# WangChangqi98/CSS

Measured on AMD Instinct MI355X. Metric: training images/sec at 513x513 R101-DeepLabv3+ (mix_label step, labeled+unlabeled crops consumed), higher is better.
Workload: dtype bf16

## Files before the change

### css_amd/csrc/abi.hip

```cpp
#include "../../include/css_hip.h"
#include "launchers.h"

#include <cstdlib>
#include <cstring>
#include <mutex>
#include <new>
#include <vector>

namespace {
inline hipStream_t S(css_stream_t s) { return reinterpret_cast<hipStream_t>(s); }
inline void set_dev(int device) {
  if (device >= 0) (void)hipSetDevice(device);
}
int g_cu_count[64] = {0};
int cu_count(int device) {
  int d = device;
  if (d < 0) (void)hipGetDevice(&d);
  if (d < 0 || d >= 64) return 256;
  if (!g_cu_count[d]) {
    int v = 0;
    if (hipDeviceGetAttribute(&v, hipDeviceAttributeMultiprocessorCount, d) != hipSuccess || v <= 0) v = 256;
    g_cu_count[d] = v;
  }
  return g_cu_count[d];
// ... 147 lines not shown
int css_conv2d_dgrad(const void* dy, const void* w_t, void* dx, int N, int H, int W, int Cin, int lddx, int Ho, int Wo, int Cout, int lddy, int R,
                     int Sk, int stride, int pad, int dil, double alg_flops, int dtype, int device, css_stream_t stream) {
  set_dev(device);
  if (stride != 1 && stride != 2) return CSS_ERR_ARG;
  ConvArgs a = {};
  a.src = dy; a.wt = w_t; a.dst = dx; a.bias = nullptr;
  a.N = N; a.Hs = Ho; a.Ws = Wo; a.Cs = Cout; a.lds = lddy;
  a.Hd = H; a.Wd = W; a.Cd = Cin; a.ldd = lddx;
  a.R = R; a.S = Sk; a.stride = stride; a.pad = pad; a.dil = dil; a.mode = 1;
  a.M = N * H * W; a.Ktot = R * Sk * Cout;
  ConvProf cp(1, 6, alg_flops, S(stream));
  cp.ws_bytes = conv1x1_bytes(a, dtype);
  cp.conv_bytes = conv_alg_bytes(a, dtype);
  return css_launch_conv(a, dtype, cu_count(device), S(stream), g_prof_on ? &cp : nullptr);
}
static int dgrad_add_impl(const void* dy, const void* w_t, void* dx, const void* addend, int ld_add, const unsigned char* mask, int N, int H, int W, int Cin,
                          int lddx, int Ho, int Wo, int Cout, int lddy, int R, int Sk, int stride, int pad, int dil, double alg_flops, int dtype,
                          int device, css_stream_t stream) {
  set_dev(device);
  if (stride != 1 && stride != 2) return CSS_ERR_ARG;
  if (mask) {
    const int vec = dtype == CSS_BF16 ? 8 : 4;
    if (!addend || (Cin % vec) || (lddx % vec) || (ld_add % vec) || (reinterpret_cast<uintptr_t>(dx) & 15) || (reinterpret_cast<uintptr_t>(addend) & 15))
      return CSS_ERR_ARG;
  }
  ConvArgs a = {};
  a.src = dy; a.wt = w_t; a.dst = dx; a.bias = nullptr;
  a.N = N; a.Hs = Ho; a.Ws = Wo; a.Cs = Cout; a.lds = lddy;
  a.Hd = H; a.Wd = W; a.Cd = Cin; a.ldd = lddx;
  a.R = R; a.S = Sk; a.stride = stride; a.pad = pad; a.dil = dil; a.mode = 1; a.addend = addend; a.ld_add = ld_add; a.add_mask = mask;
  a.M = N * H * W; a.Ktot = R * Sk * Cout;
  ConvProf cp(1, 6, alg_flops, S(stream));
  cp.ws_bytes = conv1x1_bytes(a, dtype);
  cp.conv_bytes = conv_alg_bytes(a, dtype);
  return css_launch_conv(a, dtype, cu_count(device), S(stream), g_prof_on ? &cp : nullptr);
}
int css_conv2d_dgrad_add(const void* dy, const void* w_t, void* dx, const void* addend, int ld_add, int N, int H, int W, int Cin, int lddx, int Ho, int Wo, int Cout, int lddy, int R,
                     int Sk, int stride, int pad, int dil, double alg_flops, int dtype, int device, css_stream_t stream) {
  return dgrad_add_impl(dy, w_t, dx, addend, ld_add, nullptr, N, H, W, Cin, lddx, Ho, Wo, Cout, lddy, R, Sk, stride, pad, dil, alg_flops, dtype, device, stream);
}
int css_conv2d_dgrad_add_masked(const void* dy, const void* w_t, void* dx, const void* addend, int ld_add, const unsigned char* mask, int N, int H, int W, int Cin,
                                int lddx, int Ho, int Wo, int Cout, int lddy, int R, int Sk, int stride, int pad, int dil, double alg_flops, int dtype,
                                int device, css_stream_t stream) {
  if (!mask) return CSS_ERR_ARG;
  return dgrad_add_impl(dy, w_t, dx, addend, ld_add, mask, N, H, W, Cin, lddx, Ho, Wo, Cout, lddy, R, Sk, stride, pad, dil, alg_flops, dtype, device, stream);
}
size_t css_conv2d_wgrad_ws_bytes(int M, int Ktot, int Cout, int dtype, int device) {
  return css_wgrad_ws_bytes_(M, Ktot, Cout, dtype, cu_count(device));
}
int css_conv2d_wgrad(const void* x, const void* dy, float* dw, float* ws, size_t ws_bytes, int N, int H, int W, int Cin, int ldx, int Ho, int Wo,
                     int Cout, int lddy, int R, int Sk, int stride, int pad, int dil, double alg_flops, int dtype, int device,
                     css_stream_t stream) {
  set_dev(device);
  WgradArgs a;
  a.ws = ws; a.ws_bytes = ws ? ws_bytes : 0;
  a.x = x; a.dy = dy; a.dw = dw;
  a.N = N; a.Hs = H; a.Ws = W; a.Cs = Cin; a.ldx = ldx;
  a.Hd = Ho; a.Wd = Wo; a.Cd = Cout; a.ldy = lddy;
  a.R = R; a.S = Sk; a.stride = stride; a.pad = pad; a.dil = dil;
  a.M = N * Ho * Wo; a.Ktot = R * Sk * Cin; a.m_per_split = a.M;
  ConvProf cp(2, 7, alg_flops, S(stream));
  return css_launch_wgrad(a, dtype, cu_count(device), S(stream), g_prof_on ? &cp : nullptr);
}
int css_conv_ws_applies(int M, int K, int ld_src, int N, int ld_dst, int R, int Sk, int stride, int pad, int has_stats, int has_addend, int ld_add,
                        int has_bias, int dtype, int n_cu) {
  static const bool no_dma = getenv("CSS_NO_DMA_CONV") != nullptr, no_256 = getenv("CSS_NO_DMA256_CONV") != nullptr;
  if (dtype != CSS_BF16 || no_dma || no_256) return 0;
  alignas(16) static float dummy[4];
  ConvArgs a = {};
  a.N = 1; a.Hs = a.Hd = 1; a.Ws = a.Wd = M; a.M = M;
  a.Cs = K; a.lds = ld_src; a.Cd = N; a.ldd = ld_dst; a.Ktot = R * Sk * K;
  a.R = R; a.S = Sk; a.stride = stride; a.pad = pad; a.dil = 1;
  a.stats = has_stats ? dummy : nullptr;
  a.addend = has_addend ? dummy : nullptr; a.ld_add = ld_add;
  a.bias = has_bias ? dummy : nullptr;
  return css_conv_ws_supported(a, n_cu > 0 ? n_cu : 256) ? 1 : 0;
}
int css_conv_c64_applies(int N, int H, int W, int Cin, int ld_src, int Cout, int ld_dst, int R, int Sk, int stride, int pad, int dil, int has_addend,
                         int has_bias, int dtype) {
  static const bool no_dma = getenv("CSS_NO_DMA_CONV") != nullptr;
  if (no_dma) return 0;
  alignas(16) static float dummy[4];
  ConvArgs a = {};
  a.N = N; a.Hs = a.Hd = H; a.Ws = a.Wd = W; a.M = N * H * W;
  a.Cs = Cin; a.lds = ld_src; a.Cd = Cout; a.ldd = ld_dst; a.Ktot = R * Sk * Cin;
  a.R = R; a.S = Sk; a.stride = stride; a.pad = pad; a.dil = dil;
  a.src = a.wt = dummy; a.dst = dummy;
  a.addend = has_addend ? dummy : nullptr;
  a.bias = has_bias ? dummy : nullptr;
  return css_conv_c64_supported(a, dtype) ? 1 : 0;
}
int css_conv_c64_set_enabled(int on) { return css_conv_c64_set_enabled_(on); }
int css_wgrad_splits(int M, int Ktot, int Cout, int dtype, int n_cu) {
  int splits = 0, mps = 0;
  css_wgrad_plan_(M, Ktot, Cout, dtype, n_cu > 0 ? n_cu : 256, &splits, &mps);
  return splits;
}
int css_weight_layout(const float* w, void* out, int Cout, int taps, int Cin, int CinPad, int dgrad, int dtype, int device, css_stream_t stream) {
  set_dev(device);
  return css_launch_weight_layout(w, out, Cout, taps, Cin, CinPad, dgrad, dtype, S(stream));
}

int css_weight_dgrad_layout_batched(const float* flat, void* out, const long* desc, int n_layers, long total_tiles, int dtype, int device,
                                    css_stream_t stream) {
  set_dev(device);
  return css_launch_weight_dgrad_layout_batched(flat, out, desc, n_layers, total_tiles, dtype, S(stream));
}

int css_bn_nrb(int Mg, int G, int C, int dtype) { return css_bn_nrb_(Mg, G, C, dtype); }
int css_bn_stats(const void* y, int Mg, int G, int C, int ld, double* partial, int dtype, int device, css_stream_t stream) {
  set_dev(device);
  return css_launch_bn_stats(y, Mg, G, C, ld, partial, dtype, S(stream));
}
int css_bn_reduce(const double* partial, int nrb, int C, int G, double* sums, float* dgamma, float* dbeta, int accumulate, double count_local,
                  int device, css_stream_t stream) {
  set_dev(device);
  return css_launch_bn_reduce(partial, nrb, C, G, sums, dgamma, dbeta, accumulate, count_local, S(stream));
}
int css_bn_reduce_finalize(const double* partial, int nrb, int G, double count, const float* gamma, const float* beta, float* running_mean,
                           float* running_var, float momentum, float eps, float* mean, float* invstd, float* scale, float* shift, int C,
                           int device, css_stream_t stream) {
  set_dev(device);
  return css_launch_bn_reduce_finalize(partial, nrb, G, count, gamma, beta, running_mean, running_var, momentum, eps, mean, invstd, scale, shift,
                                       C, S(stream));
}
int css_bn_reduce_finalize_slabs(const float* partial, int M, int Mg, int G, double count, const float* gamma, const float* beta,
                                 float* running_mean, float* running_var, float momentum, float eps, float* mean, float* invstd, float* scale,
                                 float* shift, double* sums_out, int C, const void* y, int ldy, int tile_rows, int device, css_stream_t stream) {
  set_dev(device);
  return css_launch_bn_reduce_slabs(partial, M, Mg, G, count, gamma, beta, running_mean, running_var, momentum, eps, mean, invstd, scale, shift,
                                    sums_out, C, y, ldy, tile_rows, S(stream));
}
int css_bn_finalize(const double* sums, int G, double count, const double* count_dev, const float* gamma, const float* beta, float* running_mean,
                    float* running_var, float momentum, float eps, float* mean, float* invstd, float* scale, float* shift, int C, int device,
                    css_stream_t stream) {
  set_dev(device);
  return css_launch_bn_finalize(sums, G, count, count_dev, gamma, beta, running_mean, running_var, momentum, eps, mean, invstd, scale, shift, C, S(stream));
}
int css_peer_alloc(size_t bytes, int device, void** out, int* mem_kind_out) {
  if (!out || bytes == 0) return CSS_ERR_ARG;
  set_dev(device);
  void* p = nullptr;
  int kind = 1;
  if (hipExtMallocWithFlags(&p, bytes, hipDeviceMallocFinegrained) != hipSuccess || !p) {
    (void)hipGetLastError();
// ... 316 lines not shown
```

### css_amd/csrc/common.h

```cpp
#pragma once
#include <hip/hip_runtime.h>
#include <stdint.h>

typedef __bf16 bf16_t;
typedef __attribute__((ext_vector_type(8))) __bf16 bf16x8;
typedef __attribute__((ext_vector_type(4))) __bf16 bf16x4;
typedef __attribute__((ext_vector_type(4))) short s16x4;
typedef __attribute__((ext_vector_type(16))) float f32x16;
typedef __attribute__((ext_vector_type(4))) float f32x4;

enum { CSS_F32 = 0, CSS_BF16 = 1 };

enum {
  CSS_OK = 0,
  CSS_ERR_ARG = -1,
  CSS_ERR_DTYPE = -2,
  CSS_ERR_LAUNCH = -3,
  CSS_ERR_WORKSPACE = -4
};

#define CSS_CHECK_LAUNCH()                                   \
  do {                                                       \
    hipError_t e__ = hipGetLastError();                      \
    if (e__ != hipSuccess) return CSS_ERR_LAUNCH;            \
// ... 12 lines not shown
  }
  uint32_t lg = 31 - __builtin_clz(d);
  if (d & (d - 1)) lg += 1;
  uint32_t p = 31 + lg;
  f.mul = (uint32_t)((((uint64_t)1 << p) + d - 1) / d);
  f.shr = p - 32;
  return f;
}
__device__ __forceinline__ uint32_t fdiv(uint32_t n, const FastDiv& f) {
  return f.d <= 1 ? n : (__umulhi(n, f.mul) >> f.shr);
}

template <typename T> struct ElemT;
template <> struct ElemT<float> {
  static constexpr int VEC = 4;
  static __device__ __forceinline__ float to_f(float v) { return v; }
  static __device__ __forceinline__ float from_f(float v) { return v; }
};
template <> struct ElemT<bf16_t> {
  static constexpr int VEC = 8;
  static __device__ __forceinline__ float to_f(bf16_t v) { return (float)v; }
  static __device__ __forceinline__ bf16_t from_f(float v) { return (bf16_t)v; }
};

template <typename T> struct Vec16 {
  static constexpr int N = 16 / sizeof(T);
  union {
    uint4 raw;
    T e[N];
    uint32_t w[4];
  };
  __device__ __forceinline__ Vec16() {}
  __device__ __forceinline__ void zero() { raw = make_uint4(0, 0, 0, 0); }
  __device__ __forceinline__ void load(const T* p) { raw = *reinterpret_cast<const uint4*>(p); }
  __device__ __forceinline__ void store(T* p) const { *reinterpret_cast<uint4*>(p) = raw; }
  typedef __attribute__((ext_vector_type(4))) unsigned int nt_u32x4;
  __device__ __forceinline__ void load(const T* p, bool nt) {
    if (nt) {
      const nt_u32x4 t = __builtin_nontemporal_load(reinterpret_cast<const nt_u32x4*>(p));
      raw = make_uint4(t[0], t[1], t[2], t[3]);
    } else {
      load(p);
    }
  }
  __device__ __forceinline__ void store(T* p, bool nt) const {
    if (nt) {
      const nt_u32x4 t = {raw.x, raw.y, raw.z, raw.w};
      __builtin_nontemporal_store(t, reinterpret_cast<nt_u32x4*>(p));
    } else {
      store(p);
    }
  }
  __device__ __forceinline__ void store_sc1(T* p) const {
    const nt_u32x4 t = {raw.x, raw.y, raw.z, raw.w};
    asm volatile("global_store_dwordx4 %0, %1, off sc1" ::"v"(p), "v"(t) : "memory");
  }
  __device__ __forceinline__ float f(int i) const { return ElemT<T>::to_f(e[i]); }
  __device__ __forceinline__ void set(int i, float v) { e[i] = ElemT<T>::from_f(v); }
};

typedef __attribute__((ext_vector_type(2))) float f32x2;
typedef __attribute__((ext_vector_type(2))) bf16_t bf16x2_pk;
__device__ __forceinline__ unsigned pack2_bf16(float lo, float hi) {
  return __builtin_bit_cast(unsigned, __builtin_convertvector(f32x2{lo, hi}, bf16x2_pk));
}
template <typename T> struct Pairs;
template <> struct Pairs<float> {
  static constexpr int NP = 2;
  static __device__ __forceinline__ f32x2 get(const Vec16<float>& v, int p) { return f32x2{v.e[2 * p], v.e[2 * p + 1]}; }
  static __device__ __forceinline__ void set(Vec16<float>& v, int p, f32x2 x) { v.e[2 * p] = x[0]; v.e[2 * p + 1] = x[1]; }
};
template <> struct Pairs<bf16_t> {
  static constexpr int NP = 4;
  static __device__ __forceinline__ f32x2 get(const Vec16<bf16_t>& v, int p) {
    return f32x2{__builtin_bit_cast(float, v.w[p] << 16), __builtin_bit_cast(float, v.w[p] & 0xffff0000u)};
  }
  static __device__ __forceinline__ void set(Vec16<bf16_t>& v, int p, f32x2 x) { v.w[p] = pack2_bf16(x[0], x[1]); }
};
__device__ __forceinline__ float keep_if_bit(float x, unsigned bits, int b) {
  return __builtin_bit_cast(float, __builtin_bit_cast(unsigned, x) & (unsigned)__builtin_amdgcn_sbfe((int)bits, b, 1));
}

__device__ __forceinline__ unsigned keep_mask_bf16x2(unsigned bits, int w) {
  return ((unsigned)__builtin_amdgcn_sbfe((int)bits, 2 * w, 1) & 0xFFFFu) | ((unsigned)__builtin_amdgcn_sbfe((int)bits, 2 * w + 1, 1) & 0xFFFF0000u);
}

__device__ __forceinline__ float wave_sum(float v) {
#pragma unroll
  for (int o = 32; o > 0; o >>= 1) v += __shfl_xor(v, o, 64);
  return v;
}
__device__ __forceinline__ float wave_max(float v) {
#pragma unroll
  for (int o = 32; o > 0; o >>= 1) v = fmaxf(v, __shfl_xor(v, o, 64));
  return v;
}

typedef __attribute__((ext_vector_type(4))) unsigned int u32x4;
constexpr unsigned OOB = 0x80000000u;
__device__ __forceinline__ uint4 bload16(__amdgpu_buffer_rsrc_t r, unsigned off) {
  u32x4 v = __builtin_amdgcn_raw_buffer_load_b128(r, (int)off, 0, 0);
  return make_uint4(v[0], v[1], v[2], v[3]);
}
typedef __attribute__((address_space(3))) void lds_void;

static inline int cdiv(long a, long b) { return (int)((a + b - 1) / b); }
```

### css_amd/csrc/conv.hip

```cpp
#include "common.h"
#include "launchers.h"
#include <cstdlib>

template <typename T> struct Mma;
template <> struct Mma<bf16_t> {
  static constexpr int KS = 16;
  typedef bf16x8 frag;
  static __device__ __forceinline__ frag load(const bf16_t* row_k, int h) {
    return *reinterpret_cast<const frag*>(row_k + h * 8);
  }
  static __device__ __forceinline__ f32x16 mma(frag a, frag b, f32x16 c) {
    return __builtin_amdgcn_mfma_f32_32x32x16_bf16(a, b, c, 0, 0, 0);
  }
};
template <> struct Mma<float> {
  static constexpr int KS = 2;
  typedef float frag;
  static __device__ __forceinline__ frag load(const float* row_k, int h) { return row_k[h]; }
  static __device__ __forceinline__ f32x16 mma(frag a, frag b, f32x16 c) {
    return __builtin_amdgcn_mfma_f32_32x32x2f32(a, b, c, 0, 0, 0);
  }
};

template <int CV>
// ... 676 lines not shown
  }
}
static void launch_small_n128(dim3 g, hipStream_t st, const ConvArgs& b, int n_cu = 0) {
  static const bool dma = !(getenv("CSS_SMALL_DMA") && atoi(getenv("CSS_SMALL_DMA")) == 0) && !getenv("CSS_NO_DMA_CONV");
  static const int nst2 = getenv("CSS_SMALL_NST2") ? atoi(getenv("CSS_SMALL_NST2")) : 1;
  if (dma && b.Cs % 64 == 0 && nst2 && n_cu > 0 && (int)g.x > n_cu) {
    hipLaunchKernelGGL((conv_igemm_dma_kernel<128, 128, 2, 2, 2>), g, dim3(256), 0, st, b);
  } else if (dma && b.Cs % 64 == 0) {
    hipLaunchKernelGGL((conv_igemm_dma_kernel<128, 128, 2, 2>), g, dim3(256), 0, st, b);
  } else {
    hipLaunchKernelGGL((conv_igemm_kernel<bf16_t, 128, 128, 64, 2, 2>), g, dim3(256), 0, st, b);
  }
}

enum ConvPlan { PLAN_OTHER = 0, PLAN_WS = 1, PLAN_TILE256 = 3 };
static ConvPlan conv_plan(const ConvArgs& a, int dtype, int n_cu) {
  static const bool no_dma = getenv("CSS_NO_DMA_CONV") != nullptr, no_256 = getenv("CSS_NO_DMA256_CONV") != nullptr;
  if (dtype != CSS_BF16 || no_dma || no_256) return PLAN_OTHER;
  if (css_conv_ws_supported(a, n_cu)) return PLAN_WS;
  if (a.Cd >= 256 && css_conv_pp_plan(a, n_cu) != 0) return PLAN_TILE256;
  return PLAN_OTHER;
}
int css_conv_tile_rows_(const ConvArgs& a, int dtype, int n_cu) { (void)a; (void)dtype; (void)n_cu; return 256; }

int css_launch_conv(const ConvArgs& a_in, int dtype, int n_cu, hipStream_t st, LaunchProf* prof) {
  auto P0 = [&](bool big, double share, bool ws = false) { if (prof) prof->begin(big, share, ws); };
  auto P1 = [&]() { if (prof) prof->end(); };
  ConvArgs a = a_in;
  a.m_begin = 0;
  {
    static const int conv_nt = getenv("CSS_CONV_NT") ? atoi(getenv("CSS_CONV_NT")) & 3 : 0;
    a.st_nt = conv_nt;
  }
  if (a.M <= 0 || a.Cd <= 0) return CSS_OK;
  if (a.stats && (dtype != CSS_BF16 || a.stat_Mg < 128 || a.addend)) return CSS_ERR_ARG;
  a.stat_nslab = cdiv(a.M, 128);
  a.stat_G = a.stats ? a.M / a.stat_Mg : 0;
  {
    const size_t esz = dtype == CSS_BF16 ? 2 : 4;
    const size_t sb = (size_t)a.N * a.Hs * a.Ws * a.lds * esz, wb = (size_t)a.Cd * a.Ktot * esz;
    if (sb >= 0x7FFFFFF0ull || wb >= 0x7FFFFFF0ull) return CSS_ERR_ARG;
    a.src_bytes = (unsigned)sb;
    a.wt_bytes = (unsigned)wb;
  }
  if (dtype == CSS_BF16) {
    if (a.Cs % 8 || a.lds % 8 || (reinterpret_cast<uintptr_t>(a.src) & 15) || (reinterpret_cast<uintptr_t>(a.wt) & 15))
      return CSS_ERR_ARG;
    static const bool no_dma = getenv("CSS_NO_DMA_CONV") != nullptr;
    const ConvPlan plan = conv_plan(a, dtype, n_cu);
    if (!no_dma && css_conv_c64_supported(a, dtype)) {
      P0(false, 1.0);
      css_launch_conv_c64(a, n_cu, st);
      P1();
    } else if (plan == PLAN_WS) {
      P0(true, 1.0, true);
      css_launch_conv_ws(a, n_cu, st);
      P1();
    } else if (plan == PLAN_TILE256) {
      const int nt_n = cdiv(a.Cd, 256), mt = cdiv(a.M, 256);
      int full_mt = mt;
      const double rounds = (double)mt * nt_n / n_cu;
      if (rounds > 1.0 && rounds - (long)rounds < 0.6 && (rounds - (long)rounds) > 1e-9) full_mt = (int)((long)rounds * n_cu / nt_n);
      if (full_mt > 0) {
        ConvArgs b = a;
        b.M = full_mt * 256 < a.M ? full_mt * 256 : a.M;
        P0(true, (double)(b.M - b.m_begin) / a.M);
        {
          b.dst_bytes = (unsigned)((size_t)b.M * b.ldd * 2);
          const int tiles = full_mt * nt_n;
          if (css_conv_p8_supported(b)) css_launch_conv_p8(b, tiles < n_cu ? tiles : n_cu, st);
          else css_launch_conv_pp(b, tiles < n_cu ? tiles : n_cu, st);
        }
        P1();
      }
      if (full_mt < mt) {
        ConvArgs b = a;
        b.m_begin = full_mt * 256;
        P0(false, (double)(b.M - b.m_begin) / a.M);
        {
          static const int rem_mode = getenv("CSS_REM_N64") ? atoi(getenv("CSS_REM_N64")) : 1;
          const int wgs128 = cdiv(a.M - b.m_begin, 128) * cdiv(a.Cd, 128);
          if ((rem_mode == 1 && wgs128 * 2 <= n_cu) || (rem_mode == 2 && wgs128 <= n_cu))
            launch_small_n64(dim3(cdiv(a.M - b.m_begin, 128) * cdiv(a.Cd, 64)), st, b, n_cu, true);
          else
            launch_small_n128(dim3(wgs128), st, b, n_cu);
        }
        P1();
      }
    } else if (a.Cd > 64 && !no_dma) {
      const int nt_n = cdiv(a.Cd, 128), mt = cdiv(a.M, 256);
      const int slots = n_cu;
      static const bool small_only = !(getenv("CSS_N128_SMALL_ONLY") && atoi(getenv("CSS_N128_SMALL_ONLY")) == 0);
      int full_mt = small_only ? 0 : mt;
      const double rounds = (double)mt * nt_n / slots;
      if (!small_only && rounds > 1.0 && rounds - (long)rounds < 0.6 && (rounds - (long)rounds) > 1e-9) {
        full_mt = (int)((long)rounds * slots / nt_n);
      }
      if (full_mt > 0) {
        ConvArgs b = a;
        b.M = full_mt * 256 < a.M ? full_mt * 256 : a.M;
        P0(false, (double)(b.M - b.m_begin) / a.M);
        hipLaunchKernelGGL((conv_igemm_dma_kernel<256, 128, 4, 2>), dim3(full_mt * nt_n), dim3(512), 0, st, b);
        P1();
      }
      if (full_mt < mt) {
        ConvArgs b = a;
// ... 31 lines not shown
```

### css_amd/csrc/launchers.h

```cpp
#pragma once
#include "common.h"

struct ConvArgs {
  const void* src;
  const void* wt;
  void* dst;
  const float* bias;
  int N, Hs, Ws, Cs, lds;
  int Hd, Wd, Cd, ldd;
  int R, S, stride, pad, dil;
  int mode;
  int M, Ktot;
  unsigned src_bytes, wt_bytes;
  int m_begin;
  float* stats;
  int stat_Mg, stat_nslab;
  int stat_G;
  const void* addend;
  int ld_add;
  const unsigned char* add_mask;
  unsigned dst_bytes;
  FastDiv fd_hw, fd_w;
  unsigned stat_bytes, add_bytes;
  unsigned mask_bytes;
  int korder;
  int tab_da[63], tab_kb[63], tab_tap[63];
  int st_nt;
};

struct WgradArgs {
  const void* x;
  const void* dy;
  float* dw;
  int N, Hs, Ws, Cs, ldx;
  int Hd, Wd, Cd, ldy;
  int R, S, stride, pad, dil;
  int M, Ktot, m_per_split;
  FastDiv fd_hw, fd_w;
  unsigned x_bytes, dy_bytes;
  int splits, tiles_k, tiles_n;
  float* ws;
  size_t ws_bytes;
  int nt;
  int compact;
  int row_lo[3], row_n[3], row_mps[3];
  int cls_nrows[2], cls_rows[2][3];
  FastDiv fd_L[3];
};


struct LaunchProf {
  virtual void begin(bool big, double share, bool ws) = 0;
  virtual void end() = 0;
};
int css_launch_conv(const ConvArgs& a, int dtype, int n_cu, hipStream_t st, LaunchProf* prof = nullptr);
int css_launch_wgrad(WgradArgs a, int dtype, int n_cu, hipStream_t st, LaunchProf* prof = nullptr);
bool css_conv_pp_supported(const ConvArgs& a);
bool css_conv_c64_supported(const ConvArgs& a, int dtype);
void css_launch_conv_c64(ConvArgs a, int n_cu, hipStream_t st);
int css_conv_c64_set_enabled_(int on);
int css_conv_pp_plan(const ConvArgs& a, int n_cu);
void css_launch_conv_pp(ConvArgs a, int grid, hipStream_t st);
int css_conv_tile_rows_(const ConvArgs& a, int dtype, int n_cu);
bool css_conv_p8_supported(const ConvArgs& a);
void css_launch_conv_p8(ConvArgs a, int grid, hipStream_t st);
bool css_conv_ws_supported(const ConvArgs& a, int n_cu);
void css_launch_conv_ws(ConvArgs a, int n_cu, hipStream_t st);
void css_conv_ws_set_enabled(int on);
void css_wgrad_plan_(int M, int Ktot, int Cd, int dtype, int n_cu, int* splits_out, int* mps_out);
size_t css_wgrad_ws_bytes_(int M, int Ktot, int Cd, int dtype, int n_cu);

int css_stem_s2d_enabled_();
int css_stem_s2d_tile_rows_();
int css_launch_nchw_to_s2d(const float* x, void* out, int N, int C, int H, int W, hipStream_t st);
int css_launch_stem_s2d_weights(const float* w, void* out, int Cout, int R, hipStream_t st);
int css_launch_stem_s2d_fold_wgrad(const float* dw2, float* dw, int Cout, int R, hipStream_t st);
int css_launch_conv_stem_s2d(const void* x, const void* w2, void* y, float* stats, int Mg, int N, int Hs, int Ws, int Cout, int R, int n_cu,
                             hipStream_t st);

int css_bn_nrb_(int Mg, int G, int C, int dtype);
int css_launch_bn_stats(const void* y, int Mg, int G, int C, int ld, double* partial, int dtype, hipStream_t st);
int css_launch_bn_reduce(const double* partial, int nrb, int C, int G, double* sums, float* g1, float* g0, int accumulate, double count_local,
                         hipStream_t st);
int css_launch_bn_reduce_finalize(const double* partial, int nrb, int G, double count, const float* gamma, const float* beta,
                                  float* running_mean, float* running_var, float momentum, float eps, float* mean, float* invstd, float* scale,
                                  float* shift, int C, hipStream_t st);
int css_launch_bn_reduce_slabs(const float* partial, int M, int Mg, int G, double count, const float* gamma, const float* beta,
                               float* running_mean, float* running_var, float momentum, float eps, float* mean, float* invstd, float* scale,
                               float* shift, double* sums_out, int C, const void* y, int ldy, int tile_rows, hipStream_t st);
int css_launch_bn_finalize(const double* sums, int G, double count, const double* count_dev, const float* gamma, const float* beta,
                           float* running_mean, float* running_var, float momentum, float eps, float* mean, float* invstd, float* scale,
                           float* shift, int C, hipStream_t st);
int css_launch_bn_eval_coeff(const float* gamma, const float* beta, const float* rm, const float* rv, float eps, float* scale, float* shift, int C,
                             hipStream_t st);
int css_launch_bn_apply(const void* y, int ldy, const void* res, int ldr, void* out, int ldo, const float* scale, const float* shift, int M, int C,
                        int relu, int Mg, unsigned char* mask, int dtype, hipStream_t st);
int css_launch_bn_apply_pool(const void* y, void* out, uint8_t* arg, const float* scale, const float* shift, int N, int H, int W, int C, int Ho, int Wo,
                             int G, int relu, int dtype, hipStream_t st);
int css_launch_bn_bwd_reduce(const void* da, int ldda, const void* a, int lda, const void* y, int ldy, const float* mean, const float* invstd,
                             const float* scale, const float* shift, int Mg, int G, int C, int relu, double* partial, const unsigned char* mask,
                             int dtype, hipStream_t st);
int css_launch_bn_bwd_apply(const void* da, int ldda, const void* a, int lda, const void* y, int ldy, void* dy, int lddy, void* dres, int lddr,
                            const float* mean, const float* invstd, const float* gamma, const double* sums, const float* scale, const float* shift,
                            double count, const double* count_dev, int M, int C, int relu, int Mg, const unsigned char* mask, int dtype,
                            hipStream_t st);

int css_launch_maxpool_fwd(const void* x, void* out, uint8_t* arg, int N, int H, int W, int C, int Ho, int Wo, int ks, int stride, int pad,
                           int dtype, hipStream_t st);
int css_launch_maxpool_bwd(const void* dout, const uint8_t* arg, void* dx, int N, int H, int W, int C, int Ho, int Wo, int ks, int stride, int pad,
                           int dtype, hipStream_t st);
int css_launch_bilinear(const void* x, int ldx, void* out, int ldo, int N, int Hs, int Ws, int C, int Hd, int Wd, int dtype_in, int dtype_out,
                        int backward, hipStream_t st);
int css_launch_spatial_sum(const void* x, int ldx, void* out, int N, int HW, int C, float scale, int dtype, hipStream_t st);
// ... 74 lines not shown
```

### include/css_hip.h

```cpp
#ifndef CSS_HIP_H
#define CSS_HIP_H
#include <stddef.h>
#include <stdint.h>

#ifdef __cplusplus
extern "C" {
#endif

#define CSS_API __attribute__((visibility("default")))
typedef void* css_stream_t;

#define CSS_DTYPE_F32 0
#define CSS_DTYPE_BF16 1

CSS_API int css_abi_version(void);
CSS_API int css_device_cu_count(int device);

CSS_API int css_prof_enable(int on);
CSS_API int css_prof_reset(void);
CSS_API int css_prof_read(int kind, double* total_ms, double* launches, double* alg_work);

CSS_API int css_conv2d_forward(const void* x, const void* w, const float* bias, void* y, int N, int H, int W, int Cin, int ldx, int Ho, int Wo,
                               int Cout, int ldy, int R, int S, int stride, int pad, int dil, double alg_flops, int dtype, int device,
                               css_stream_t stream);
CSS_API int css_conv2d_forward_bnstats(const void* x, const void* w, void* y, float* stats, int Mg, int N, int H, int W, int Cin, int ldx, int Ho,
                                       int Wo, int Cout, int ldy, int R, int S, int stride, int pad, int dil, double alg_flops, int dtype,
                                       int device, css_stream_t stream);
CSS_API int css_conv2d_forward_bnstats_tile_rows(const void* x, const void* w, void* y, int N, int H, int W, int Cin, int ldx, int Ho, int Wo,
                                                 int Cout, int ldy, int R, int S, int stride, int pad, int dil, int dtype, int device);
CSS_API int css_conv_ws_applies(int M, int K, int ld_src, int N, int ld_dst, int R, int S, int stride, int pad, int has_stats, int has_addend,
                                int ld_add, int has_bias, int dtype, int n_cu);
CSS_API int css_conv_c64_applies(int N, int H, int W, int Cin, int ld_src, int Cout, int ld_dst, int R, int S, int stride, int pad, int dil,
                                 int has_addend, int has_bias, int dtype);
CSS_API int css_conv_c64_set_enabled(int on);
CSS_API int css_conv2d_dgrad(const void* dy, const void* w_t, void* dx, int N, int H, int W, int Cin, int lddx, int Ho, int Wo, int Cout, int lddy,
                             int R, int S, int stride, int pad, int dil, double alg_flops, int dtype, int device, css_stream_t stream);
CSS_API int css_conv2d_dgrad_add(const void* dy, const void* w_t, void* dx, const void* addend, int ld_add, int N, int H, int W, int Cin, int lddx,
                                 int Ho, int Wo, int Cout, int lddy, int R, int S, int stride, int pad, int dil, double alg_flops, int dtype,
                                 int device, css_stream_t stream);
CSS_API int css_conv2d_dgrad_add_masked(const void* dy, const void* w_t, void* dx, const void* addend, int ld_add, const unsigned char* mask, int N,
                                        int H, int W, int Cin, int lddx, int Ho, int Wo, int Cout, int lddy, int R, int S, int stride, int pad,
                                        int dil, double alg_flops, int dtype, int device, css_stream_t stream);
CSS_API size_t css_conv2d_wgrad_ws_bytes(int M, int Ktot, int Cout, int dtype, int device);
CSS_API int css_conv2d_wgrad(const void* x, const void* dy, float* dw, float* ws, size_t ws_bytes, int N, int H, int W, int Cin, int ldx, int Ho,
                             int Wo, int Cout, int lddy, int R, int S, int stride, int pad, int dil, double alg_flops, int dtype, int device,
                             css_stream_t stream);
CSS_API int css_wgrad_splits(int M, int Ktot, int Cout, int dtype, int n_cu);
CSS_API int css_weight_layout(const float* w, void* out, int Cout, int taps, int Cin, int CinPad, int dgrad, int dtype, int device,
                              css_stream_t stream);
CSS_API int css_weight_dgrad_layout_batched(const float* flat, void* out, const long* desc, int n_layers, long total_tiles, int dtype,
                                            int device, css_stream_t stream);

CSS_API int css_bn_nrb(int Mg, int G, int C, int dtype);
CSS_API int css_bn_stats(const void* y, int Mg, int G, int C, int ld, double* partial, int dtype, int device, css_stream_t stream);
CSS_API int css_bn_reduce(const double* partial, int nrb, int C, int G, double* sums, float* dgamma, float* dbeta, int accumulate,
                          double count_local, int device, css_stream_t stream);
CSS_API int css_bn_reduce_finalize(const double* partial, int nrb, int G, double count, const float* gamma, const float* beta,
                                   float* running_mean, float* running_var, float momentum, float eps, float* mean, float* invstd, float* scale,
                                   float* shift, int C, int device, css_stream_t stream);
CSS_API int css_bn_reduce_finalize_slabs(const float* partial, int M, int Mg, int G, double count, const float* gamma, const float* beta,
                                         float* running_mean, float* running_var, float momentum, float eps, float* mean, float* invstd,
                                         float* scale, float* shift, double* sums_out, int C, const void* y, int ldy, int tile_rows,
                                         int device, css_stream_t stream);
CSS_API int css_bn_finalize(const double* sums, int G, double count, const double* count_dev, const float* gamma, const float* beta,
                            float* running_mean, float* running_var, float momentum, float eps, float* mean, float* invstd, float* scale,
                            float* shift, int C, int device, css_stream_t stream);
CSS_API int css_peer_alloc(size_t bytes, int device, void** out, int* mem_kind_out);
CSS_API int css_peer_free(void* p, int device);
CSS_API int css_peer_ipc_export(void* p, int device, unsigned char* handle64);
CSS_API int css_peer_ipc_open(const unsigned char* handle64, int device, void** out);
CSS_API int css_peer_ipc_close(void* p, int device);
CSS_API size_t css_peer_buffer_bytes(int slot_doubles);
CSS_API int css_bn_peer_finalize(const unsigned long long* bases, int world, int rank, unsigned long long seq, int slot_doubles, const double* local,
                                 int G, int C, const float* gamma, const float* beta, float* running_mean, float* running_var, float momentum,
                                 float eps, float* mean, float* invstd, float* scale, float* shift, double* count_out, int* status,
                                 long timeout_ticks, int phase, int device, css_stream_t stream);
CSS_API int css_bn_peer_gather(const unsigned long long* bases, int world, int rank, unsigned long long seq, int slot_doubles, const double* local,
                               int n, double* out, int* status, long timeout_ticks, int phase, int device, css_stream_t stream);
CSS_API int css_bn_eval_coeff(const float* gamma, const float* beta, const float* running_mean, const float* running_var, float eps, float* scale,
                              float* shift, int C, int device, css_stream_t stream);
CSS_API int css_bn_apply(const void* y, int ldy, const void* res, int ldr, void* out, int ldo, const float* scale, const float* shift, int M, int C,
                         int relu, int Mg, int dtype, int device, css_stream_t stream);
CSS_API int css_bn_apply_maxpool(const void* y, void* out, uint8_t* argmax, const float* scale, const float* shift, int N, int H, int W, int C, int Ho,
                                 int Wo, int G, int relu, int dtype, int device, css_stream_t stream);
CSS_API int css_bn_bwd_reduce(const void* da, int ldda, const void* a, int lda, const void* y, int ldy, const float* mean, const float* invstd,
                              const float* scale, const float* shift, int Mg, int G, int C, int relu, double* partial, int dtype, int device,
                              css_stream_t stream);
// ... 104 lines not shown
```

Before: 304.7.

## Add specialized persistent 3x3 conv kernel for Cin=128 with register-resident weights

Adds a dedicated bf16 3x3 stride-1 convolution kernel for 128 input channels and 64 or 128 output channels. It keeps all weights in registers (VGPR and AGPR), streams input halo rows into LDS with direct buffer-to-LDS DMA, double-buffers across persistent tiles, and can fuse BN statistics and dgrad mode. It is dispatched before the generic workspace and plan paths when its shape constraints hold. The aim is to cut the cost of the many 128-channel 3x3 convs, in exchange for heavy register pressure, low occupancy and one more specialized code path that must stay correct.

```diff
diff --git a/css_amd/csrc/abi.hip b/css_amd/csrc/abi.hip
--- a/css_amd/csrc/abi.hip
+++ b/css_amd/csrc/abi.hip
@@ -223,7 +223,7 @@
                      int Cout, int lddy, int R, int Sk, int stride, int pad, int dil, double alg_flops, int dtype, int device,
                      css_stream_t stream) {
   set_dev(device);
-  WgradArgs a;
+  WgradArgs a = {};
   a.ws = ws; a.ws_bytes = ws ? ws_bytes : 0;
   a.x = x; a.dy = dy; a.dw = dw;
   a.N = N; a.Hs = H; a.Ws = W; a.Cs = Cin; a.ldx = ldx;
@@ -262,6 +262,21 @@
   return css_conv_c64_supported(a, dtype) ? 1 : 0;
 }
 int css_conv_c64_set_enabled(int on) { return css_conv_c64_set_enabled_(on); }
+int css_conv_c128_applies(int N, int H, int W, int Cin, int ld_src, int Cout, int ld_dst, int R, int Sk, int stride, int pad, int dil, int has_addend,
+                          int has_bias, int dtype) {
+  static const bool no_dma = getenv("CSS_NO_DMA_CONV") != nullptr;
+  if (no_dma) return 0;
+  alignas(16) static float dummy[4];
+  ConvArgs a = {};
+  a.N = N; a.Hs = a.Hd = H; a.Ws = a.Wd = W; a.M = N * H * W;
+  a.Cs = Cin; a.lds = ld_src; a.Cd = Cout; a.ldd = ld_dst; a.Ktot = R * Sk * Cin;
+  a.R = R; a.S = Sk; a.stride = stride; a.pad = pad; a.dil = dil;
+  a.src = a.wt = dummy; a.dst = dummy;
+  a.addend = has_addend ? dummy : nullptr;
+  a.bias = has_bias ? dummy : nullptr;
+  return css_conv_c128_supported(a, dtype) ? 1 : 0;
+}
+int css_conv_c128_set_enabled(int on) { return css_conv_c128_set_enabled_(on); }
 int css_wgrad_splits(int M, int Ktot, int Cout, int dtype, int n_cu) {
   int splits = 0, mps = 0;
   css_wgrad_plan_(M, Ktot, Cout, dtype, n_cu > 0 ? n_cu : 256, &splits, &mps);
diff --git a/css_amd/csrc/common.h b/css_amd/csrc/common.h
--- a/css_amd/csrc/common.h
+++ b/css_amd/csrc/common.h
@@ -88,8 +88,12 @@
     }
   }
   __device__ __forceinline__ void store_sc1(T* p) const {
+#if defined(__gfx942__) || defined(__gfx950__)
     const nt_u32x4 t = {raw.x, raw.y, raw.z, raw.w};
     asm volatile("global_store_dwordx4 %0, %1, off sc1" ::"v"(p), "v"(t) : "memory");
+#else
+    store(p);
+#endif
   }
   __device__ __forceinline__ float f(int i) const { return ElemT<T>::to_f(e[i]); }
   __device__ __forceinline__ void set(int i, float v) { e[i] = ElemT<T>::from_f(v); }
diff --git a/css_amd/csrc/conv.hip b/css_amd/csrc/conv.hip
--- a/css_amd/csrc/conv.hip
+++ b/css_amd/csrc/conv.hip
@@ -752,6 +752,10 @@
       P0(false, 1.0);
       css_launch_conv_c64(a, n_cu, st);
       P1();
+    } else if (!no_dma && css_conv_c128_supported(a, dtype)) {
+      P0(false, 1.0);
+      css_launch_conv_c128(a, n_cu, st);
+      P1();
     } else if (plan == PLAN_WS) {
       P0(true, 1.0, true);
       css_launch_conv_ws(a, n_cu, st);
diff --git a/css_amd/csrc/conv_c128.hip b/css_amd/csrc/conv_c128.hip
--- /dev/null
+++ b/css_amd/csrc/conv_c128.hip
@@ -0,0 +1,295 @@
+#include "common.h"
+#include "launchers.h"
+#include <cstdlib>
+
+namespace {
+typedef __attribute__((address_space(3))) void c12_lds_void;
+constexpr unsigned C12_OOB = 0x80000000u;
+typedef __attribute__((ext_vector_type(4))) unsigned int c12_u32x4;
+typedef __attribute__((ext_vector_type(4))) float c12_f32x4;
+typedef __attribute__((ext_vector_type(2))) float c12_f32x2;
+
+__device__ __forceinline__ void c12_dma16(__amdgpu_buffer_rsrc_t r, void* lds_wave_base, unsigned off) {
+  __builtin_amdgcn_raw_ptr_buffer_load_lds(r, (c12_lds_void*)lds_wave_base, 16, (int)off, 0, 0, 0);
+}
+__device__ __forceinline__ float c12_row16_sum(float v) {
+  v += __builtin_bit_cast(float, __builtin_amdgcn_update_dpp(0, __builtin_bit_cast(int, v), 0x128, 0xf, 0xf, false));
+  v += __builtin_bit_cast(float, __builtin_amdgcn_update_dpp(0, __builtin_bit_cast(int, v), 0x124, 0xf, 0xf, false));
+  v += __builtin_bit_cast(float, __builtin_amdgcn_update_dpp(0, __builtin_bit_cast(int, v), 0x122, 0xf, 0xf, false));
+  v += __builtin_bit_cast(float, __builtin_amdgcn_update_dpp(0, __builtin_bit_cast(int, v), 0x121, 0xf, 0xf, false));
+  return v;
+}
+__device__ __forceinline__ void c12_swap16(unsigned& a, unsigned& b) {
+  asm volatile("s_nop 1\n\tv_permlane16_swap_b32 %0, %1" : "+v"(a), "+v"(b));
+}
+__device__ __forceinline__ float c12_lo(unsigned u) { return __builtin_bit_cast(float, u << 16); }
+__device__ __forceinline__ float c12_hi(unsigned u) { return __builtin_bit_cast(float, u & 0xffff0000u); }
+template <int N> __device__ __forceinline__ void c12_wait_vm() { asm volatile("s_waitcnt vmcnt(%0)" ::"n"(N) : "memory"); }
+}
+
+template <int NWC, bool STATS, bool DGRAD>
+__global__ __launch_bounds__(256) void conv3x3_c128_kernel(const ConvArgs a) {
+  constexpr int BT = 128, HT = 64, NWP = 4 / NWC, PXW = HT / NWP, NI = PXW / 16;
+  constexpr int NPI = 17, RB = NPI * 1024, NPIECE = 3 * NPI, NPWV = 13;
+  constexpr int BUF = 4 * NPWV * 1024;
+  constexpr int KB = 36;
+  constexpr int NSET = NI == 4 ? 3 : 5;
+  static_assert(NPWV * 4 >= NPIECE && 3 * RB <= BUF && 4 * NPI >= HT + 2 && 2 * NPWV <= KB, "pieces per wave");
+  __shared__ __attribute__((aligned(1024))) unsigned char smem[2 * BUF + (STATS ? 4 * 64 * 4 : 0)];
+
+  const int tid = threadIdx.x, lane = tid & 63;
+  const int wave = __builtin_amdgcn_readfirstlane(tid >> 6);
+  const int cg = wave % NWC, pg = wave / NWC;
+  const int l15 = lane & 15, lg = lane >> 4;
+  const int W = a.Wd, H = a.Hd, M = a.M, Cd = 32 * NWC;
+  const int ntiles = (M + BT - 1) / BT;
+  const int G = gridDim.x, q8 = G >> 3, r8 = G & 7;
+  const int xcd = blockIdx.x & 7, idx8 = blockIdx.x >> 3;
+  const int pos0 = (xcd < r8 ? xcd * (q8 + 1) : r8 * (q8 + 1) + (xcd - r8) * q8) + idx8;
+  if (pos0 >= ntiles) return;
+
+  unsigned long long src_p = (unsigned long long)a.src, wt_p = (unsigned long long)a.wt;
+  int src_n = (int)a.src_bytes, wt_n = (int)a.wt_bytes;
+  asm volatile("" : "+s"(src_p), "+s"(wt_p), "+s"(src_n), "+s"(wt_n));
+  const __amdgpu_buffer_rsrc_t rs_a = __builtin_amdgcn_make_buffer_rsrc((void*)src_p, 0, src_n, 0x00020000);
+  const __amdgpu_buffer_rsrc_t rs_b = __builtin_amdgcn_make_buffer_rsrc((void*)wt_p, 0, wt_n, 0x00020000);
+  const __amdgpu_buffer_rsrc_t rs_d = __builtin_amdgcn_make_buffer_rsrc(a.dst, 0, (int)a.dst_bytes, 0x00020000);
+
+  bf16x8 fw[KB][2];
+#pragma unroll
+  for (int q = 0; q < KB; ++q)
+#pragma unroll
+    for (int j = 0; j < 2; ++j) {
+      const unsigned off = ((unsigned)(32 * cg + 16 * j + l15) * 1152u + (unsigned)(32 * q + 8 * lg)) * 2u;
+      fw[q][j] = __builtin_bit_cast(bf16x8, __builtin_amdgcn_raw_buffer_load_b128(rs_b, (int)off, 0, 0));
+    }
+
+  const unsigned lds2 = (unsigned)a.lds * 2u;
+  auto issue_piece = [&](int i, int t, int half, int buf) {
+    const int p = wave * NPWV + i;
+    const int ar = p / NPI, c = p - NPI * ar;
+    const int pos = 4 * c + (lane >> 4);
+    const int P = t * BT + half * HT + (ar - 1) * W - 1 + pos;
+    const bool ok = p < NPIECE && t < ntiles && P >= 0 && P < M;
+#ifndef C12_ABL_NODMA
+    c12_dma16(rs_a, smem + buf * BUF + p * 1024, ok ? (unsigned)P * lds2 + (unsigned)(((lane & 15) ^ (pos & 15)) * 16) : C12_OOB);
+#else
+    (void)ok; (void)buf;
+#endif
+  };
+  int t = pos0, half = 0;
+  __builtin_amdgcn_sched_barrier(0);
+#pragma unroll
+  for (int i = 0; i < NPWV; ++i) issue_piece(i, t, 0, 0);
+  __builtin_amdgcn_sched_barrier(0);
+#pragma unroll
+  for (int q = 0; q < KB; ++q)
+#pragma unroll
+    for (int j = 0; j < 2; ++j) {
+      if (j == 0) asm volatile("" : "+v"(fw[q][j]));
+      else asm volatile("" : "+a"(fw[q][j]));
+    }
+  c12_wait_vm<0>();
+
+  int lb[3];
+#pragma unroll
+  for (int b = 0; b < 3; ++b) lb[b] = (l15 + b) * 256 + ((lg ^ ((l15 + b) & 15)) << 4);
+  f32x4 acc[NI][2];
+  const int nl = 32 * cg + 16 * (lg & 1) + 8 * (lg >> 1);
+  float* const carry = reinterpret_cast<float*>(smem + 2 * BUF);
+  c12_f32x2 s01[2], s23[2], q01[2], q23[2];
+  int cur = 0;
+
+  for (;;) {
+    const int m0s = t * BT, m0 = m0s + half * HT, mw = m0 + PXW * pg;
+    unsigned vm[NI];
+#pragma unroll
+    for (int i = 0; i < NI; ++i) {
+      const int m = mw + 16 * i + l15;
+      const int n = (int)fdiv((uint32_t)m, a.fd_hw), r = m - n * (H * W);
+      const int y = (int)fdiv((uint32_t)r, a.fd_w), x = r - y * W;
+      unsigned yb = 0, xb = 0;
+#pragma unroll
+      for (int e = 0; e < 3; ++e) {
+        yb |= (unsigned)(y - 1 + e >= 0 && y - 1 + e < H) << e;
+        xb |= (unsigned)(x - 1 + e >= 0 && x - 1 + e < W) << e;
+      }
+      unsigned v = 0;
+#pragma unroll
+      for (int e = 0; e < 3; ++e) v |= ((yb >> e) & 1u) ? (xb << (3 * e)) : 0u;
+      if (m >= M) v = 0;
+#ifdef C12_ABL_NOVALID
+      v = (unsigned)(lane + i) | 0x1FFu;
+#endif
+      vm[i] = v;
+    }
+    __builtin_amdgcn_sched_barrier(0);
+    if (STATS && half == 0) c12_wait_vm<NI + 4>();
+    else c12_wait_vm<NI>();
+    __builtin_amdgcn_s_barrier();
+    asm volatile("" ::: "memory");
+    __builtin_amdgcn_sched_barrier(0);
+    const int t_next = half ? t + G : t;
+
+    const unsigned char* const pb = smem + cur * BUF + (PXW * pg) * 256;
+    auto read_frag = [&](int q, int i, bf16x8& f) {
+      const int tp = DGRAD ? 8 - (q >> 2) : (q >> 2), ar = tp / 3, b = tp - 3 * ar, cq = q & 3;
+      f = *reinterpret_cast<const bf16x8*>(pb + (lb[b] ^ (cq << 6)) + ar * RB + i * 4096);
+    };
+    auto mask_frag = [&](int q, int i, bf16x8& f) {
+      const int tp = DGRAD ? 8 - (q >> 2) : (q >> 2);
+      const bool ok = (vm[i] >> tp) & 1u;
+      c12_u32x4 u = __builtin_bit_cast(c12_u32x4, f);
+#pragma unroll
+      for (int e = 0; e < 4; ++e) u[e] = ok ? u[e] : 0u;
+      f = __builtin_bit_cast(bf16x8, u);
+    };
+    {
+      bf16x8 fa[NSET][NI];
+#pragma unroll
+      for (int q = 0; q < NSET; ++q)
+#pragma unroll
+        for (int i = 0; i < NI; ++i) read_frag(q, i, fa[q][i]);
+#pragma unroll
+      for (int i = 0; i < NI; ++i) mask_frag(0, i, fa[0][i]);
+      __builtin_amdgcn_sched_barrier(0);
+      const f32x4 z = {0.f, 0.f, 0.f, 0.f};
+#pragma unroll
+      for (int q = 0; q < KB; ++q)
+#pragma unroll
+        for (int i = 0; i < NI; ++i) {
+#pragma unroll
+#ifndef C12_ABL_NOMFMA
+          for (int j = 0; j < 2; ++j) acc[i][j] = __builtin_amdgcn_mfma_f32_16x16x32_bf16(fw[q][j], fa[q % NSET][i], q == 0 ? z : acc[i][j], 0, 0, 0);
+#else
+          for (int j = 0; j < 2; ++j) { if (q == 0) acc[i][j] = z; asm volatile("" ::"v"(fa[q % NSET][i])); }
+#endif
+          if (q + NSET < KB) read_frag(q + NSET, i, fa[q % NSET][i]);
+          if (q + 1 < KB) mask_frag(q + 1, i, fa[(q + 1) % NSET][i]);
+          if (i == NI - 1 && q % 2 == 0 && q / 2 < NPWV) issue_piece(q / 2, t_next, half ^ 1, cur ^ 1);
+          __builtin_amdgcn_sched_barrier(0);
+        }
+    }
+    cur ^= 1;
+
+    const int bnd = STATS ? (m0s / a.stat_Mg + 1) * a.stat_Mg : 0x7fffffff;
+    const bool whole = m0s + BT <= bnd;
+    if (STATS && half == 0) {
+#pragma unroll
+      for (int j = 0; j < 2; ++j) s01[j] = s23[j] = q01[j] = q23[j] = c12_f32x2{0.f, 0.f};
+    }
+    auto out_tiles = [&](bool test) {
+#pragma unroll
+      for (int i = 0; i < NI; ++i) {
+        const int m = mw + 16 * i + l15;
+        unsigned lo[2], hi[2];
+#pragma unroll
+        for (int j = 0; j < 2; ++j) {
+          lo[j] = pack2_bf16(acc[i][j][0], acc[i][j][1]);
+          hi[j] = pack2_bf16(acc[i][j][2], acc[i][j][3]);
+          if (STATS) {
+            c12_f32x2 v01 = {c12_lo(lo[j]), c12_hi(lo[j])}, v23 = {c12_lo(hi[j]), c12_hi(hi[j])};
+            if (test && !(m < bnd)) { v01 = c12_f32x2{0.f, 0.f}; v23 = c12_f32x2{0.f, 0.f}; }
+            s01[j] += v01; s23[j] += v23;
+            q01[j] += v01 * v01; q23[j] += v23 * v23;
+          }
+        }
+        c12_swap16(lo[0], lo[1]);
+        c12_swap16(hi[0], hi[1]);
+        const c12_u32x4 vv = {lo[0], hi[0], lo[1], hi[1]};
+#ifdef C12_ABL_NOSTORE
+        __builtin_amdgcn_raw_buffer_store_b128(vv, rs_d, (int)C12_OOB, 0, 0);
+#else
+        __builtin_amdgcn_raw_buffer_store_b128(vv, rs_d, (int)(m < M ? ((unsigned)m * (unsigned)a.ldd + (unsigned)nl) * 2u : C12_OOB), 0, 0);
+#endif
+      }
+    };
+    if (!STATS || whole) out_tiles(false);
+    else out_tiles(true);
+    if (STATS && half == 1) {
+      c12_f32x4 o[2][2];
+#pragma unroll
+      for (int j = 0; j < 2; ++j) {
+        o[j][0] = c12_f32x4{c12_row16_sum(s01[j][0]), c12_row16_sum(s01[j][1]), c12_row16_sum(s23[j][0]), c12_row16_sum(s23[j][1])};
+        o[j][1] = c12_f32x4{c12_row16_sum(q01[j][0]), c12_row16_sum(q01[j][1]), c12_row16_sum(q23[j][0]), c12_row16_sum(q23[j][1])};
+      }
+      float* const cw = carry + wave * 64;
+      if (l15 == 0) {
+#pragma unroll
+        for (int j = 0; j < 2; ++j)
+#pragma unroll
+          for (int sq = 0; sq < 2; ++sq) *reinterpret_cast<c12_f32x4*>(cw + ((j * 2 + sq) * 4 + lg) * 4) = o[j][sq];
+      }
+      asm volatile("s_waitcnt lgkmcnt(0)" ::: "memory");
+      __builtin_amdgcn_s_barrier();
+      asm volatile("" ::: "memory");
+      const __amdgpu_buffer_rsrc_t rs_s = __builtin_amdgcn_make_buffer_rsrc(a.stats, 0, (int)a.stat_bytes, 0x00020000);
+      const unsigned base = (unsigned)(m0s >> 7) * 2u * (unsigned)Cd * 4u;
+      const bool lane_ok = pg == 0 && l15 == 0;
+#pragma unroll
+      for (int j = 0; j < 2; ++j)
+#pragma unroll
+        for (int sq = 0; sq < 2; ++sq) {
+          c12_f32x4 tsum = {0.f, 0.f, 0.f, 0.f};
+          if (lane_ok) {
+            tsum = *reinterpret_cast<const c12_f32x4*>(carry + cg * 64 + ((j * 2 + sq) * 4 + lg) * 4);
+#pragma unroll
+            for (int g2 = 1; g2 < NWP; ++g2)
+              tsum += *reinterpret_cast<const c12_f32x4*>(carry + (g2 * NWC + cg) * 64 + ((j * 2 + sq) * 4 + lg) * 4);
+          }
+          const int n = sq * Cd + 32 * cg + 16 * j + 4 * lg;
+          __builtin_amdgcn_raw_buffer_store_b128(__builtin_bit_cast(c12_u32x4, tsum), rs_s, (int)(lane_ok ? base + (unsigned)n * 4u : C12_OOB), 0, 0);
+        }
+    }
+    __builtin_amdgcn_sched_barrier(0);
+    t = t_next;
+    half ^= 1;
+    if (t >= ntiles) break;
+  }
+  asm volatile("s_waitcnt vmcnt(0)" ::: "memory");
+}
+
+static int g_c128_off = -1;
+static void c128_read_env() {
+  if (g_c128_off < 0) {
+    const char* e = getenv("CSS_NO_C128_CONV");
+    g_c128_off = (e && *e && !(e[0] == '0' && !e[1])) ? 1 : 0;
+  }
+}
+int css_conv_c128_set_enabled_(int on) {
+  c128_read_env();
+  const int was = g_c128_off ? 0 : 1;
+  g_c128_off = on ? 0 : 1;
+  return was;
+}
+bool css_conv_c128_supported(const ConvArgs& a, int dtype) {
+  c128_read_env();
+  if (g_c128_off || dtype != CSS_BF16) return false;
+  if (a.R != 3 || a.S != 3 || a.stride != 1 || a.pad != 1 || a.dil != 1 || a.Hs != a.Hd || a.Ws != a.Wd) return false;
+  if (a.Cs != 128 || a.Ktot != 1152 || (a.Cd != 64 && a.Cd != 128) || a.addend || a.bias || a.m_begin != 0) return false;
+  if (a.lds % 8 || a.lds < 128 || a.ldd % 8 || (reinterpret_cast<uintptr_t>(a.src) & 15) || (reinterpret_cast<uintptr_t>(a.wt) & 15) ||
+      (reinterpret_cast<uintptr_t>(a.dst) & 15))
+    return false;
+  if (a.M != a.N * a.Hd * a.Wd || a.M <= 0) return false;
+  if ((size_t)a.M * a.lds * 2 >= 0x7FFFFFF0ull || (size_t)a.M * a.ldd * 2 >= 0x7FFFFFF0ull) return false;
+  if (a.stats && a.stat_Mg < 128) return false;
+  if (a.mode && a.stats) return false;
+  return true;
+}
+void css_launch_conv_c128(ConvArgs a, int n_cu, hipStream_t st) {
+  a.dst_bytes = (unsigned)((size_t)a.M * a.ldd * 2);
+  if (a.stats) a.stat_bytes = (unsigned)((size_t)2 * cdiv(a.M, 256) * 2 * a.Cd * 4);
+  a.fd_hw = make_fastdiv((uint32_t)(a.Hd * a.Wd));
+  a.fd_w = make_fastdiv((uint32_t)a.Wd);
+  const int ntiles = cdiv(a.M, 128);
+  const dim3 g(ntiles < n_cu ? ntiles : n_cu), b(256);
+  if (a.Cd == 64) {
+    if (a.mode) hipLaunchKernelGGL((conv3x3_c128_kernel<2, false, true>), g, b, 0, st, a);
+    else if (a.stats) hipLaunchKernelGGL((conv3x3_c128_kernel<2, true, false>), g, b, 0, st, a);
+    else hipLaunchKernelGGL((conv3x3_c128_kernel<2, false, false>), g, b, 0, st, a);
+  } else {
+    if (a.mode) hipLaunchKernelGGL((conv3x3_c128_kernel<4, false, true>), g, b, 0, st, a);
+    else if (a.stats) hipLaunchKernelGGL((conv3x3_c128_kernel<4, true, false>), g, b, 0, st, a);
+    else hipLaunchKernelGGL((conv3x3_c128_kernel<4, false, false>), g, b, 0, st, a);
+  }
+}
diff --git a/css_amd/csrc/launchers.h b/css_amd/csrc/launchers.h
--- a/css_amd/csrc/launchers.h
+++ b/css_amd/csrc/launchers.h
@@ -59,6 +59,9 @@
 bool css_conv_c64_supported(const ConvArgs& a, int dtype);
 void css_launch_conv_c64(ConvArgs a, int n_cu, hipStream_t st);
 int css_conv_c64_set_enabled_(int on);
+bool css_conv_c128_supported(const ConvArgs& a, int dtype);
+void css_launch_conv_c128(ConvArgs a, int n_cu, hipStream_t st);
+int css_conv_c128_set_enabled_(int on);
 int css_conv_pp_plan(const ConvArgs& a, int n_cu);
 void css_launch_conv_pp(ConvArgs a, int grid, hipStream_t st);
 int css_conv_tile_rows_(const ConvArgs& a, int dtype, int n_cu);
diff --git a/include/css_hip.h b/include/css_hip.h
--- a/include/css_hip.h
+++ b/include/css_hip.h
@@ -33,6 +33,9 @@
 CSS_API int css_conv_c64_applies(int N, int H, int W, int Cin, int ld_src, int Cout, int ld_dst, int R, int S, int stride, int pad, int dil,
                                  int has_addend, int has_bias, int dtype);
 CSS_API int css_conv_c64_set_enabled(int on);
+CSS_API int css_conv_c128_applies(int N, int H, int W, int Cin, int ld_src, int Cout, int ld_dst, int R, int S, int stride, int pad, int dil,
+                                  int has_addend, int has_bias, int dtype);
+CSS_API int css_conv_c128_set_enabled(int on);
 CSS_API int css_conv2d_dgrad(const void* dy, const void* w_t, void* dx, int N, int H, int W, int Cin, int lddx, int Ho, int Wo, int Cout, int lddy,
                              int R, int S, int stride, int pad, int dil, double alg_flops, int dtype, int device, css_stream_t stream);
 CSS_API int css_conv2d_dgrad_add(const void* dy, const void* w_t, void* dx, const void* addend, int ld_add, int N, int H, int W, int Cin, int lddx,
```

New measurement: 305.0 (median of 3 runs). No clear change (+0.1%).
